# merbanan/rtl_433

Hardware: NVIDIA H100
Metric: IQ MS/s end-to-end demod+slice (higher is better)
Workload: dtype u8/int16/int32 fixed point

## Files before the change

### rtl_433_b200/csrc/r433b_api.cu

```cuda
#include <algorithm>
#include <cmath>
#include <cstdio>
#include <cstdlib>
#include <chrono>
#include <cstring>
#include <exception>
#include <atomic>
#include <mutex>
#include <string>
#include <thread>
#include <vector>

#include "../../include/r433b.h"
#include "../../include/r433b_abi.h"
#include "r433b_kernels.cuh"
#include "r433b_host.hpp"
#include "r433b_pulses.hpp"
#include "r433b_analyze.cuh"
#include "r433b_analyze_host.hpp"
#include "r433b_grab.cuh"

using namespace r433b;

#ifdef R433B_SIMT_EMU
#define R4_LAUNCH(kernel, grid, block, smem, stream, ...) simt::launch(dim3(grid), dim3(block), (size_t)(smem), kernel, __VA_ARGS__)
#else
#define R4_LAUNCH(kernel, grid, block, smem, stream, ...) kernel<<<(grid), (block), (smem), (stream)>>>(__VA_ARGS__)
#endif

static_assert(sizeof(struct bitbuffer) == 6604, "bitbuffer_t layout");
static_assert(sizeof(struct pulse_data) == 9672, "pulse_data_t layout");
static_assert(sizeof(struct r_device) == 152, "r_device layout");
static_assert(offsetof(struct bitbuffer, bb) == 204, "bitbuffer_t.bb offset");

namespace {

struct DevBuf {
    void *p = nullptr;
    size_t cap = 0;
};

struct HostBuf {
    void *p = nullptr;
    size_t cap = 0;
};

}

struct r433b_ctx {
    int device = 0;
    std::string err;
    std::mutex err_mu;
    int use_mag = 0;
    float level_limit = 0.0f, min_level = -12.1442f, min_snr = 9.0f, fm_low_pass = 0.0f;
    std::vector<r433b_device> devs;
    std::vector<r433b_gate> gates;
    r433b_batch batch{};
    std::vector<uint64_t> offsets, lengths;
    bool processed = false, fetched = false;
    unsigned fpdm = 0;
    int enable_fm = 0;
    int n_sms = 132;
    int spoil_front = 0;
    size_t min_caps[3] = {0, 0, 0};
    Levels lv{};
    DevBuf d_data, d_offsets, d_train, d_pkgs, d_ppool, d_gpool, d_counters, d_am, d_fm;
    DevBuf d_devparams, d_lists, d_pairs, d_arena, d_cursor;
    size_t pkg_cap = 0, pool_cap = 0, arena_cap = 0;
    unsigned n_ook = 0, n_fsk = 0;
    unsigned n_pkgs = 0, pool_used = 0;
    unsigned long long event_bytes = 0, n_events = 0, n_samples = 0, n_gated = 0;
    HostBuf h_pkgs, h_ppool, h_gpool, h_pairs, h_events;
    r433b_timing timing{};
    cudaEvent_t ev[6]{};
    int pipeline_groups = 0;
    cudaStream_t s_in = nullptr, s_det = nullptr, s_out = nullptr;
    static constexpr int kMaxGroups = 16;
    cudaEvent_t ev_in[kMaxGroups]{}, ev_det[kMaxGroups]{}, ev_slc[kMaxGroups]{}, ev_t[4 * kMaxGroups]{}, ev_f[kMaxGroups]{}, ev_init = nullptr;
    DevBuf d_order;
    DevBuf d_sort, d_copy;
    DevBuf d_ranges, d_state, d_lengths, d_stage, d_raw, d_log, d_amoff, d_chunks, d_tiles;
    std::vector<uint64_t> am_offsets;
    HostBuf h_ranges;
    bool d2h_done = false;
    bool pulse_mode = false;
    std::vector<PulseSet::Meta> pulse_meta;
    std::vector<uint32_t> dev_index;
    bool analyzed = false;
    std::vector<r433b_analysis> an;
    std::vector<r433b_guess> an_guess;
    std::vector<std::string> an_text;
    std::vector<r433b_pair> an_pairs;
    std::vector<uint8_t> an_events;
    DevBuf d_an, d_an_dev, d_an_gap, d_an_pairs, d_an_arena;
    std::thread worker;
    bool in_flight = false;
    int worker_rc = 0;
    r433b_batch sub_batch{};
    std::vector<uint64_t> sub_offsets, sub_lengths;
    r433b_results sub_res{};
    uint8_t const *grab_src = nullptr;
    unsigned grab_flip = 0;
    std::vector<uint32_t> p_events;
    std::vector<uint8_t> dispatched;
    std::vector<r433b_grab> grabs;
    std::vector<int64_t> grab_newest;
    bool grab_planned = false;
    uint64_t grab_pushed = 0;
    uint64_t grab_prior_bytes = 0;
    std::vector<uint64_t> grab_cum;
    DevBuf d_grab_prior, d_grab_segs, d_grab_stage;
    bool chained = false;
    std::vector<uint64_t> chain_base;
    std::vector<r433b_chain *> chains;
};

struct ChainSettings {
    uint32_t sample_format, samp_rate, center_frequency, fpdm, block_bytes;
    int use_mag, enable_fm;
    float level_limit, min_level, min_snr, fm_low_pass;
    bool operator==(ChainSettings const &o) const
    {
        return sample_format == o.sample_format && samp_rate == o.samp_rate && center_frequency == o.center_frequency
                && fpdm == o.fpdm && block_bytes == o.block_bytes && use_mag == o.use_mag && enable_fm == o.enable_fm
                && level_limit == o.level_limit && min_level == o.min_level && min_snr == o.min_snr
                && fm_low_pass == o.fm_low_pass;
    }
};

struct r433b_chain {
    r433b_ctx *ctx = nullptr;
    uint32_t n = 0;
    DevBuf d_state, d_train, d_state_copy, d_train_copy, d_flags, d_base;
    std::vector<uint8_t> open;
    std::vector<uint64_t> next;
    std::vector<uint64_t> base;
    ChainSettings settings{};
};

struct r433b_pulses {
    PulseSet set;
};

namespace {
void chain_free_device(r433b_chain *ch)
{
    for (DevBuf *b : {&ch->d_state, &ch->d_train, &ch->d_state_copy, &ch->d_train_copy, &ch->d_flags, &ch->d_base}) {
        if (b->p) cudaFree(b->p);
        b->p = nullptr;
        b->cap = 0;
    }
}
}

namespace {

int fail(r433b_ctx *c, int code, char const *what, cudaError_t e = cudaSuccess)
{
    if (c) {
        std::lock_guard<std::mutex> lock(c->err_mu);
        c->err = what;
        if (e != cudaSuccess) {
            c->err += ": ";
            c->err += cudaGetErrorString(e);
        }
    }
    return code;
}

#define CU(call)                                                   \
    do {                                                           \
        cudaError_t e_ = (call);                                   \
        if (e_ != cudaSuccess) return fail(ctx, R433B_ECUDA, #call, e_); \
    } while (0)

unsigned dp_flip_of(uint32_t sample_format) { return sample_format == R433B_FMT_CS8 ? 0x80808080u : 0u; }

int dev_reserve(r433b_ctx *ctx, DevBuf &b, size_t bytes)
{
    if (bytes <= b.cap) return 0;
    if (b.p) cudaFree(b.p);
    b.p = nullptr;
    b.cap = 0;
#ifdef R433B_EXACT_ALLOC
    size_t want = bytes;
#else
    size_t want = bytes + bytes / 8 + 256;
#endif
    cudaError_t e = cudaMalloc(&b.p, want);
    if (e != cudaSuccess) return fail(ctx, R433B_ENOMEM, "cudaMalloc", e);
    b.cap = want;
    return 0;
}

int host_reserve(r433b_ctx *ctx, HostBuf &b, size_t bytes)
{
    if (bytes <= b.cap) return 0;
    if (b.p) cudaFreeHost(b.p);
    b.p = nullptr;
    b.cap = 0;
    size_t want = bytes + bytes / 8 + 256;
    cudaError_t e = cudaMallocHost(&b.p, want);
    if (e != cudaSuccess) return fail(ctx, R433B_ENOMEM, "cudaMallocHost", e);
    b.cap = want;
    return 0;
}

}

extern "C" {

int r433b_create(int cuda_device, r433b_ctx **out)
{
    if (!out) return R433B_EINVAL;
    *out = nullptr;
    int n = 0;
    cudaError_t e = cudaGetDeviceCount(&n);
    if (e != cudaSuccess || n <= 0 || cuda_device < 0 || cuda_device >= n) {
        fprintf(stderr, "r433b_create: no usable CUDA device %d (%s); there is no CPU fallback\n", cuda_device,
                e != cudaSuccess ? cudaGetErrorString(e) : "device count is 0 or index out of range");
        return R433B_ECUDA;
    }
    r433b_ctx *ctx = new (std::nothrow) r433b_ctx();
    if (!ctx) return R433B_ENOMEM;
    ctx->device = cuda_device;
    if (cudaSetDevice(cuda_device) != cudaSuccess) {
        delete ctx;
        return R433B_ECUDA;
    }
    cudaFuncSetAttribute((void const *)k_front<2>, cudaFuncAttributePreferredSharedMemoryCarveout, 100);
    cudaFuncSetAttribute((void const *)k_front<4>, cudaFuncAttributePreferredSharedMemoryCarveout, 100);
    cudaFuncSetAttribute((void const *)k_detect<2>, cudaFuncAttributePreferredSharedMemoryCarveout, 100);
    cudaFuncSetAttribute((void const *)k_detect<4>, cudaFuncAttributePreferredSharedMemoryCarveout, 100);
    cudaFuncSetAttribute((void const *)k_slice2, cudaFuncAttributePreferredSharedMemoryCarveout,
                         (int)((kSliceCtasPerSm * (sizeof(g_slice_win) + sizeof(g_slice_seg) + 1024) * 100 + 228 * 1024 - 1) / (228 * 1024)));
    for (auto &v : ctx->ev) cudaEventCreate(&v);
    cudaStreamCreateWithFlags(&ctx->s_in, cudaStreamNonBlocking);
    cudaStreamCreateWithFlags(&ctx->s_det, cudaStreamNonBlocking);
    cudaStreamCreateWithFlags(&ctx->s_out, cudaStreamNonBlocking);
    for (auto &v : ctx->ev_in) cudaEventCreateWithFlags(&v, cudaEventDisableTiming);
    for (auto &v : ctx->ev_det) cudaEventCreateWithFlags(&v, cudaEventDisableTiming);
    for (auto &v : ctx->ev_slc) cudaEventCreateWithFlags(&v, cudaEventDisableTiming);
    for (auto &v : ctx->ev_t) cudaEventCreate(&v);
    for (auto &v : ctx->ev_f) cudaEventCreate(&v);
    cudaEventCreateWithFlags(&ctx->ev_init, cudaEventDisableTiming);
    ctx->lv = compute_levels(0, 0.0f, -12.1442f, 9.0f);
    if (char const *v = getenv("R433B_SPOIL_FRONT")) ctx->spoil_front = atoi(v);
    if (char const *v = getenv("R433B_TEST_CAPS")) {
        unsigned long long c[3] = {0, 0, 0};
        sscanf(v, "%llu,%llu,%llu", &c[0], &c[1], &c[2]);
        for (int i = 0; i < 3; ++i) ctx->min_caps[i] = (size_t)c[i];
    }
    if (cudaDeviceGetAttribute(&ctx->n_sms, cudaDevAttrMultiProcessorCount, cuda_device) != cudaSuccess || ctx->n_sms <= 0)
        ctx->n_sms = 132;
    *out = ctx;
    return R433B_OK;
}

void r433b_destroy(r433b_ctx *ctx)
{
    if (!ctx) return;
    if (ctx->worker.joinable()) ctx->worker.join();
    cudaSetDevice(ctx->device);
    for (r433b_chain *ch : ctx->chains) {
        chain_free_device(ch);
        ch->ctx = nullptr;
    }
    for (DevBuf *b : {&ctx->d_data, &ctx->d_offsets, &ctx->d_train, &ctx->d_pkgs, &ctx->d_ppool, &ctx->d_gpool,
                 &ctx->d_counters, &ctx->d_am, &ctx->d_fm, &ctx->d_devparams, &ctx->d_lists, &ctx->d_pairs,
                 &ctx->d_arena, &ctx->d_cursor, &ctx->d_ranges, &ctx->d_state, &ctx->d_lengths, &ctx->d_stage, &ctx->d_raw, &ctx->d_log, &ctx->d_amoff, &ctx->d_chunks, &ctx->d_tiles,
                 &ctx->d_order, &ctx->d_sort, &ctx->d_copy, &ctx->d_an, &ctx->d_an_dev, &ctx->d_an_gap, &ctx->d_an_pairs, &ctx->d_an_arena,
                 &ctx->d_grab_prior, &ctx->d_grab_segs, &ctx->d_grab_stage})
        if (b->p) cudaFree(b->p);
    for (HostBuf *b : {&ctx->h_pkgs, &ctx->h_ppool, &ctx->h_gpool, &ctx->h_pairs, &ctx->h_events, &ctx->h_ranges})
        if (b->p) cudaFreeHost(b->p);
    for (auto &v : ctx->ev)
        if (v) cudaEventDestroy(v);
    for (auto *arr : {ctx->ev_in, ctx->ev_det, ctx->ev_slc})
        for (int i = 0; i < r433b_ctx::kMaxGroups; ++i)
            if (arr[i]) cudaEventDestroy(arr[i]);
    for (auto &v : ctx->ev_t)
        if (v) cudaEventDestroy(v);
    for (auto &v : ctx->ev_f)
        if (v) cudaEventDestroy(v);
    if (ctx->ev_init) cudaEventDestroy(ctx->ev_init);
    for (cudaStream_t st : {ctx->s_in, ctx->s_det, ctx->s_out})
        if (st) cudaStreamDestroy(st);
    delete ctx;
}

char const *r433b_last_error(r433b_ctx const *ctx) { return ctx ? ctx->err.c_str() : "no context"; }

int r433b_set_levels(r433b_ctx *ctx, int use_mag_est, float level_limit_db, float min_level_db, float min_snr_db)
{
    if (!ctx) return R433B_EINVAL;
    ctx->use_mag = use_mag_est ? 1 : 0;
    ctx->level_limit = level_limit_db;
    ctx->min_level = min_level_db;
    ctx->min_snr = min_snr_db;
    ctx->lv = compute_levels(ctx->use_mag, level_limit_db, min_level_db, min_snr_db);
    return R433B_OK;
}

int r433b_set_fm_low_pass(r433b_ctx *ctx, float v)
{
    if (!ctx) return R433B_EINVAL;
    ctx->fm_low_pass = v;
    return R433B_OK;
}

int r433b_set_pipeline(r433b_ctx *ctx, int groups)
{
    if (!ctx || groups < 0 || groups > r433b_ctx::kMaxGroups) return R433B_EINVAL;
    ctx->pipeline_groups = groups;
    return R433B_OK;
}

int r433b_set_devices(r433b_ctx *ctx, r433b_device const *devs, uint32_t n)
{
    if (!ctx || (n && !devs)) return R433B_EINVAL;
    ctx->devs.assign(devs, devs + n);
    ctx->gates.clear();
    return R433B_OK;
}

int r433b_set_gates(r433b_ctx *ctx, r433b_gate const *gates, uint32_t n)
{
    if (!ctx || (n && !gates)) return R433B_EINVAL;
    if (n && n != ctx->devs.size()) return fail(ctx, R433B_EINVAL, "r433b_set_gates: one gate per registered device");
    for (uint32_t i = 0; i < n; ++i)
        if (gates[i].code_single > 0 || gates[i].code_single < -4 || gates[i].code_multi > 0 || gates[i].code_multi < -4)
            return fail(ctx, R433B_EINVAL, "r433b_set_gates: codes are decode_fn returns 0 .. -4");
    ctx->gates.assign(gates, gates + n);
    return R433B_OK;
}

uint64_t r433b_get_gated(r433b_ctx const *ctx) { return ctx && ctx->processed ? ctx->n_gated : 0; }

int r433b_set_r_devices(r433b_ctx *ctx, struct r_device *const *devs, uint32_t n)
{
    if (!ctx || (n && !devs)) return R433B_EINVAL;
    ctx->devs.resize(n);
    ctx->gates.clear();
    for (uint32_t i = 0; i < n; ++i) {
        struct r_device const *d = devs[i];
        r433b_device &o = ctx->devs[i];
        o.modulation = d->modulation;
        o.short_width = d->short_width;
        o.long_width = d->long_width;
        o.reset_limit = d->reset_limit;
        o.gap_limit = d->gap_limit;
        o.sync_width = d->sync_width;
        o.tolerance = d->tolerance;
        o.priority = d->priority;
    }
    return R433B_OK;
}

namespace {

int upload_slicer_tables(r433b_ctx *ctx, std::vector<uint32_t> const &rates, cudaStream_t st)
{
    size_t const n_devs = ctx->devs.size();
    std::vector<SlicerParams> sp(rates.size() * n_devs);
    for (size_t g = 0; g < rates.size(); ++g)
        for (size_t i = 0; i < n_devs; ++i) {
            sp[g * n_devs + i] = scale_device(ctx->devs[i], rates[g]);
            if (!ctx->gates.empty()) sp[g * n_devs + i].gate = ctx->gates[i].min_bits;
        }
    std::vector<unsigned> lists = slice_list(ctx->devs, 1), fsk = slice_list(ctx->devs, 2);
    ctx->n_ook = (unsigned)lists.size();
    ctx->n_fsk = (unsigned)fsk.size();
    lists.insert(lists.end(), fsk.begin(), fsk.end());
    if (int r = dev_reserve(ctx, ctx->d_devparams, std::max<size_t>(1, sp.size()) * sizeof(SlicerParams))) return r;
    if (int r = dev_reserve(ctx, ctx->d_lists, (lists.size() + 1) * sizeof(unsigned))) return r;
    size_t const stage_threads = (size_t)ctx->n_sms * kSliceCtasPerSm * kSliceThreads;
    if (int r = dev_reserve(ctx, ctx->d_stage, stage_threads * kStageWords * sizeof(uint32_t))) return r;
    if (!sp.empty()) CU(cudaMemcpyAsync(ctx->d_devparams.p, sp.data(), sp.size() * sizeof(SlicerParams), cudaMemcpyHostToDevice, st));
    if (!lists.empty()) CU(cudaMemcpyAsync(ctx->d_lists.p, lists.data(), lists.size() * sizeof(unsigned), cudaMemcpyHostToDevice, st));
    return R433B_OK;
}

int reserve_sort(r433b_ctx *ctx, size_t pkgs, size_t pool_entries, cudaStream_t st)
{
    size_t const cap0 = ctx->d_sort.cap;
    if (int r = dev_reserve(ctx, ctx->d_sort, (4 * kLenBins + pkgs / 32 + 3) * sizeof(unsigned))) return r;
    if (ctx->d_sort.cap != cap0) CU(cudaMemsetAsync(ctx->d_sort.p, 0, 2 * kLenBins * sizeof(unsigned), st));
    return dev_reserve(ctx, ctx->d_copy, (pool_entries + 2 * 32 * (size_t)kMaxPulses) * sizeof(PulseGap));
}

void launch_slice(r433b_ctx *ctx, GroupRange *range, unsigned n_pkgs, unsigned rate_index, cudaStream_t st)
{
    SortScratch ss;
    ss.hist = (unsigned *)ctx->d_sort.p;
    ss.fill = ss.hist + 2 * kLenBins;
    ss.base = ss.fill + 2 * kLenBins;
    ss.copy = (PulseGap *)ctx->d_copy.p;
    ss.copy_cap = std::min<size_t>(ctx->d_copy.cap / sizeof(PulseGap), 0xffffffffu);
    unsigned const n_devs = (unsigned)ctx->devs.size();
    r433b_package *pkgs = (r433b_package *)ctx->d_pkgs.p;
    SliceParams q{};
    q.pkgs = pkgs;
    q.range = range;
    q.order = (unsigned const *)ctx->d_order.p;
    q.copy = ss.copy;
    q.group_base = ss.base;
    q.dev = (SlicerParams const *)ctx->d_devparams.p + (size_t)rate_index * n_devs;
    q.n_devs = n_devs;
    q.ook_list = (unsigned const *)ctx->d_lists.p;
    q.fsk_list = q.ook_list + ctx->n_ook;
    q.n_ook = ctx->n_ook;
    q.n_fsk = ctx->n_fsk;
    q.pairs = (r433b_pair *)ctx->d_pairs.p;
    q.arena = (uint8_t *)ctx->d_arena.p;
    q.arena_cap = ctx->arena_cap;
    q.cursor = (unsigned long long *)ctx->d_cursor.p;
    q.stage = (uint32_t *)ctx->d_stage.p;
    unsigned const bgrid = (unsigned)ctx->n_sms * 2;
    R4_LAUNCH(k_bucket_count, bgrid, kBucketThreads, 0, st, range, pkgs, n_pkgs, n_devs, ss.hist);
    R4_LAUNCH(k_bucket_scan, 1, 32, 0, st, range, ss);
    R4_LAUNCH(k_bucket_scatter, bgrid, kBucketThreads, 0, st, range, (r433b_package const *)pkgs, n_pkgs, (unsigned *)ctx->d_order.p, ss,
              (int const *)ctx->d_ppool.p, (int const *)ctx->d_gpool.p);
    R4_LAUNCH(k_slice2, (unsigned)ctx->n_sms * kSliceCtasPerSm, kSliceThreads, 0, st, q);
}

int slice_ranges(r433b_ctx *ctx, std::vector<GroupRange> const &ranges, unsigned n_pkgs, size_t pool_entries, cudaStream_t st)
{
    unsigned const n_devs = (unsigned)ctx->devs.size();
    unsigned long long cursor[4] = {0, 0, 0, 0};
    ctx->timing.slice_launches = 0;
    CU(cudaEventRecord(ctx->ev[2], st));
    if (n_pkgs && n_devs) {
        size_t const pair_bytes = (size_t)n_pkgs * n_devs * sizeof(r433b_pair);
        if (int r = dev_reserve(ctx, ctx->d_pairs, pair_bytes)) return r;
        if (int r = dev_reserve(ctx, ctx->d_order, (size_t)n_pkgs * sizeof(unsigned))) return r;
        if (int r = reserve_sort(ctx, n_pkgs, pool_entries, st)) return r;
        if (int r = dev_reserve(ctx, ctx->d_ranges, ranges.size() * sizeof(GroupRange))) return r;
        if (int r = dev_reserve(ctx, ctx->d_cursor, 64)) return r;
        for (int attempt = 0; attempt < 3; ++attempt) {
            if (int r = dev_reserve(ctx, ctx->d_arena, ctx->arena_cap)) return r;
            CU(cudaMemsetAsync(ctx->d_pairs.p, 0, pair_bytes, st));
            CU(cudaMemsetAsync(ctx->d_cursor.p, 0, 64, st));
            CU(cudaMemcpyAsync(ctx->d_ranges.p, ranges.data(), ranges.size() * sizeof(GroupRange), cudaMemcpyHostToDevice, st));
            for (size_t g = 0; g < ranges.size(); ++g) {
                launch_slice(ctx, (GroupRange *)ctx->d_ranges.p + g, n_pkgs, (unsigned)g, st);
                CU(cudaGetLastError());
                ctx->timing.slice_launches++;
            }
            CU(cudaMemcpyAsync(cursor, ctx->d_cursor.p, sizeof(cursor), cudaMemcpyDeviceToHost, st));
            CU(cudaStreamSynchronize(st));
            if (!cursor[2]) break;
            ctx->arena_cap = (size_t)cursor[0] + (1u << 20);
            if (attempt == 2) return fail(ctx, R433B_EOVERFLOW, "event arena overflow");
        }
    }
    CU(cudaEventRecord(ctx->ev[3], st));
    CU(cudaEventSynchronize(ctx->ev[3]));
    cudaEventElapsedTime(&ctx->timing.slice_ms, ctx->ev[2], ctx->ev[3]);
    ctx->event_bytes = cursor[0];
    ctx->n_events = cursor[1];
    ctx->n_gated = cursor[3];
    return R433B_OK;
}

int process_iq(r433b_ctx *ctx, r433b_batch const *b, r433b_chain *ch, uint8_t const *last)
{
    if (!ctx || !b || !b->offsets || (b->n_streams && !b->data)) return fail(ctx, R433B_EINVAL, "null argument");
    if (b->sample_format != R433B_FMT_CU8 && b->sample_format != R433B_FMT_CS16 && b->sample_format != R433B_FMT_CS8
            && b->sample_format != R433B_FMT_CF32)
        return fail(ctx, R433B_EINVAL, "sample_format must be R433B_FMT_CU8, _CS8, _CS16 or _CF32");
    bool const cf32 = b->sample_format == R433B_FMT_CF32;
    unsigned const in_div = cf32 ? 2 : 1;
    if (b->samp_rate == 0) return fail(ctx, R433B_EINVAL, "samp_rate is 0");
    int const SS = (int)(b->sample_format & 0xff);
    uint32_t block_bytes = b->block_bytes ? b->block_bytes : 262144u;
    int const T = kTile;
    if (block_bytes % (uint32_t)(T * SS) != 0) return fail(ctx, R433B_EINVAL, "block_bytes must be a multiple of 2048 samples (4096 bytes of cu8, 8192 of cs16)");
    for (uint32_t i = 0; i <= b->n_streams; ++i) {
        if (b->offsets[i] % (16 * in_div)) return fail(ctx, R433B_EINVAL, "stream offsets must be multiples of 16 bytes (32 for cf32)");
        if (i && b->offsets[i] < b->offsets[i - 1]) return fail(ctx, R433B_EINVAL, "offsets not ascending");
    }
    int enable_fm = 0;
    for (auto const &d : ctx->devs)
        if (d.modulation >= 16) enable_fm = 1;
    unsigned const fpdm = b->fpdm_mode == R433B_FPDM_AUTO ? (b->center_frequency > 800000000u ? 1u : 0u) : b->fpdm_mode;
    ChainSettings const settings{b->sample_format, b->samp_rate, b->center_frequency, fpdm, block_bytes, ctx->use_mag, enable_fm,
                                 ctx->level_limit, ctx->min_level, ctx->min_snr, ctx->fm_low_pass};
    if (ch) {
        if (ch->ctx != ctx || !last) return fail(ctx, R433B_EINVAL, "r433b_process_chained: chain of another context, or no last[]");
        if (b->n_streams != ch->n) return fail(ctx, R433B_EINVAL, "r433b_process_chained: n_streams differs from the chain's");
        if (std::find(ch->open.begin(), ch->open.end(), 1) != ch->open.end() && !(settings == ch->settings))
            return fail(ctx, R433B_ESTATE, "r433b_process_chained: format, rate, frequency, block size, levels or FM "
                                           "settings changed while a file of the chain is open");
        for (uint32_t i = 0; i < b->n_streams; ++i) {
            uint64_t const in_bytes = b->lengths ? b->lengths[i] : b->offsets[i + 1] - b->offsets[i];
            if (!last[i] && in_bytes % ((uint64_t)block_bytes * in_div))
                return fail(ctx, R433B_EINVAL, "r433b_process_chained: a chunk that is not its file's last must be whole "
                                               "blocks (block_bytes, 2 x block_bytes of cf32 input)");
        }
    }
    CU(cudaSetDevice(ctx->device));
    ctx->processed = ctx->fetched = false;
    ctx->chained = false;
    ctx->pulse_mode = false;
    ctx->batch = *b;
    ctx->batch.sample_format = (uint32_t)SS;
    ctx->batch.block_bytes = block_bytes;
    ctx->offsets.assign(b->offsets, b->offsets + b->n_streams + 1);
    for (auto &v : ctx->offsets) v /= in_div;
    ctx->batch.offsets = ctx->offsets.data();
    ctx->lengths.resize(b->n_streams);
    for (uint32_t i = 0; i < b->n_streams; ++i) {
        uint64_t gap = b->offsets[i + 1] - b->offsets[i];
        ctx->lengths[i] = b->lengths ? b->lengths[i] : gap;
        if (ctx->lengths[i] > gap) return fail(ctx, R433B_EINVAL, "lengths[i] exceeds the gap to the next offset");
        if (cf32) ctx->lengths[i] = ctx->lengths[i] / 8 * 4;
    }
    ctx->batch.lengths = ctx->lengths.data();
    ctx->grabs.clear();
    ctx->grab_planned = false;
    ctx->timing.grab_ms = 0;
    uint64_t const total_bytes = b->n_streams ? b->offsets[b->n_streams] / in_div : 0;
    uint64_t used_bytes = 0;
    for (uint64_t v : ctx->lengths) used_bytes += v;
    uint32_t const n_devs = (uint32_t)ctx->devs.size();

    ctx->fpdm = fpdm;
    ctx->enable_fm = enable_fm;

    cudaStream_t const st = 0;
    ctx->d2h_done = false;

    uint8_t const *d_in;
    if (b->data_on_device && !cf32) {
        d_in = (uint8_t const *)b->data;
    } else {
        if (int r = dev_reserve(ctx, ctx->d_data, total_bytes + 64)) return r;
        d_in = (uint8_t const *)ctx->d_data.p;
    }
    ctx->grab_src = d_in;
    ctx->grab_flip = dp_flip_of(b->sample_format);
    if (cf32 && !b->data_on_device)
        if (int r = dev_reserve(ctx, ctx->d_raw, 2 * total_bytes + 64)) return r;
    if (int r = dev_reserve(ctx, ctx->d_offsets, (b->n_streams + 1) * sizeof(uint64_t))) return r;
    CU(cudaMemcpy(ctx->d_offsets.p, ctx->offsets.data(), (b->n_streams + 1) * sizeof(uint64_t), cudaMemcpyHostToDevice));
    if (int r = dev_reserve(ctx, ctx->d_lengths, std::max<size_t>(1, b->n_streams) * sizeof(uint64_t))) return r;
    if (b->n_streams) CU(cudaMemcpy(ctx->d_lengths.p, ctx->lengths.data(), b->n_streams * sizeof(uint64_t), cudaMemcpyHostToDevice));
    if (int r = dev_reserve(ctx, ctx->d_train, (size_t)std::max(1u, b->n_streams) * kTrainInts * sizeof(int))) return r;
    if (int r = dev_reserve(ctx, ctx->d_log, (size_t)std::max(1u, b->n_streams) * kLogCap * 2 * sizeof(unsigned))) return r;
    if (int r = dev_reserve(ctx, ctx->d_counters, 64)) return r;
    if (int r = dev_reserve(ctx, ctx->d_cursor, 64)) return r;
    ctx->am_offsets.resize(b->n_streams + 1);
    ctx->am_offsets[0] = 0;
    for (uint32_t i = 0; i < b->n_streams; ++i)
        ctx->am_offsets[i + 1] = ctx->am_offsets[i] + (ctx->lengths[i] / SS + T - 1) / T * T;
    uint64_t const am_samples = ctx->am_offsets[b->n_streams];
    if (int r = dev_reserve(ctx, ctx->d_am, am_samples * sizeof(int16_t) + 16)) return r;
    if (int r = dev_reserve(ctx, ctx->d_chunks, am_samples / kChunk * sizeof(ChunkInfo) + 16)) return r;
    if (int r = dev_reserve(ctx, ctx->d_tiles, am_samples / T * sizeof(TileInfo) + 16)) return r;
    if (int r = dev_reserve(ctx, ctx->d_amoff, (b->n_streams + 1) * sizeof(uint64_t))) return r;
    CU(cudaMemcpy(ctx->d_amoff.p, ctx->am_offsets.data(), (b->n_streams + 1) * sizeof(uint64_t), cudaMemcpyHostToDevice));
    if (b->want_stages)
        if (int r = dev_reserve(ctx, ctx->d_fm, total_bytes / SS * sizeof(int16_t) + 16)) return r;

    DetectParams dp{};
// ... 1287 lines not shown
```

### rtl_433_b200/csrc/r433b_host.hpp

```cpp
#pragma once
#include <algorithm>
#include <cmath>
#include <cstdint>
#include <cstring>
#include <vector>

#include "../../include/r433b.h"
#include "../../include/r433b_abi.h"
#include "r433b_core.cuh"
#include "r433b_slice.cuh"

namespace r433b {

inline Levels compute_levels(int use_mag, float level_limit, float min_level, float min_snr)
{
    Levels lv;
    if (use_mag) {
        lv.fixed_high = level_limit < 0.0 ? (int)(powf(10, (level_limit + 84.2884f) / 20.0f)) : 0;
        lv.min_high = (int)(powf(10, (min_level + 84.2884f) / 20.0f));
        lv.ratio = (int)(0.5 + powf(10, min_snr / 20.0f));
    } else {
        lv.fixed_high = level_limit < 0.0 ? (int)(powf(10, (level_limit + 42.1442f) / 10.0f)) : 0;
        lv.min_high = (int)(powf(10, (min_level + 42.1442f) / 10.0f));
        lv.ratio = (int)(0.5 + powf(10, min_snr / 10.0f));
    }
    lv.max_high = (int)(powf(10, (0 + 42.1442f) / 10.0f));
    return lv;
}

inline void fm_coeffs(int cs16, uint32_t rate, float low_pass, int &a1, int &b0)
{
    if (low_pass > 1e4f)
        low_pass = low_pass / rate;
    else if (low_pass >= 1.0f)
        low_pass = 1e6f / low_pass / rate;
    double ita = 1.0 / tan(M_PI_2 * low_pass);
    if (!cs16) {
        double gain = 1.0 / (1.0 + ita) / 2;
        a1 = (int)((ita - 1.0) * gain * 32768);
        b0 = (int)(gain * 32768);
    } else {
        double gain = 1.0 / (1.0 + ita);
        a1 = (int)((ita - 1.0) * gain * (1 << 30));
        b0 = (int)(gain * (1 << 30));
    }
}

inline SlicerParams scale_device(r433b_device const &d, uint32_t rate)
{
    SlicerParams t{};
    float per_us = rate / 1.0e6f;
    t.modulation = (int)d.modulation;
    t.s_short = d.short_width * per_us;
    t.s_long = d.long_width * per_us;
    t.s_reset = d.reset_limit * per_us;
    t.s_gap = d.gap_limit * per_us;
    t.s_sync = d.sync_width * per_us;
    t.s_tol = d.tolerance * per_us;
    bool bad3 = (d.short_width > 0 && t.s_short <= 0) || (d.long_width > 0 && t.s_long <= 0)
            || (d.reset_limit > 0 && t.s_reset <= 0);
    bool bad6 = bad3 || (d.gap_limit > 0 && t.s_gap <= 0) || (d.sync_width > 0 && t.s_sync <= 0)
            || (d.tolerance > 0 && t.s_tol <= 0);
    t.ok = (bad6 ? 0 : 1) | (bad3 ? 0 : 2);
    if ((int)d.modulation == kModOokRzi) {
        t.s_gap = t.s_sync = t.s_tol = 0;
    }
    t.f_short = d.short_width > 0.0f ? 1.0f / (d.short_width * per_us) : 0;
    t.f_long = d.long_width > 0.0f ? 1.0f / (d.long_width * per_us) : 0;
    t.priority = d.priority;
    return t;
}


inline std::vector<unsigned> slice_list(std::vector<r433b_device> const &devs, int package_type)
{
    std::vector<unsigned> v;
    for (unsigned i = 0; i < (unsigned)devs.size(); ++i)
        if (device_takes((int)devs[i].modulation, package_type)) v.push_back(i);
    std::sort(v.begin(), v.end(), [&](unsigned a, unsigned c) {
        r433b_device const &x = devs[a], &y = devs[c];
        if (x.modulation != y.modulation) return x.modulation < y.modulation;
        if (x.reset_limit != y.reset_limit) return x.reset_limit < y.reset_limit;
        if (x.short_width != y.short_width) return x.short_width < y.short_width;
        return a < c;
    });
    return v;
}


struct EventHead {
    uint32_t num_rows, dirty, free_row, len;
};

inline EventHead event_head(uint32_t h)
{
    if ((h & 0xff) == 0xff) return {1, 0, 1, 1};
    return {h & 0x7f, (h >> 7) & 1, (h >> 8) & 0xff, h >> 16};
}

template <class Row>
inline int event_rows(uint32_t const *ev, EventHead const &e, Row &&row)
{
    uint32_t const end = e.len;
    uint32_t const h = ev[0];
    if ((h & 0xff) == 0xff) {
        uint32_t const data = h >> 16, bits = (h >> 8) & 31;
        if (bits > 16) return -1;
        row(0u, bits, (h >> 13) & 7, &data, bits ? 1u : 0u);
        return 1;
    }
    uint32_t q = 1;
    for (uint32_t r = 0; r < e.num_rows && r < R433B_BITBUF_ROWS; ++r) {
        if (q + 1 > end) return -1;
        uint32_t const w = ev[q];
        q += 1;
        if (w >> 31) {
            uint32_t const data = w & 0xffff, bits = (w >> 16) & 31;
            if (bits > 16) return -1;
            row(r, bits, (w >> 21) & 0x3ff, &data, bits ? 1u : 0u);
            continue;
        }
        uint32_t const bits = w & 0xffff;
        uint32_t words = (bits + 31) / 32;
        if (e.dirty && r + 1 == e.num_rows) words = ev[end - 1];
        if (q + words > end) return -1;
        row(r, bits, w >> 16, ev + q, words);
        q += words;
    }
    return (int)q;
}

inline int event_to_bitbuffer(uint8_t const *ev8, uint32_t pair_bytes, uint32_t index, struct bitbuffer *out,
        uint32_t *consumed)
{
    if (!ev8 || !out || (pair_bytes & 3)) return -1;
    uint32_t const *ev = reinterpret_cast<uint32_t const *>(ev8);
    uint32_t const total = pair_bytes / 4;
    uint32_t pos = 0;
    EventHead e;
    for (uint32_t i = 0;; ++i) {
        if (pos + 1 > total) return -1;
        e = event_head(ev[pos]);
        if (e.len < 1 || pos + e.len > total) return -1;
        if (i == index) break;
        pos += e.len;
    }
    memset(out, 0, sizeof(*out));
    out->num_rows = (uint16_t)e.num_rows;
    out->free_row = (uint16_t)e.free_row;
    uint8_t *flat = &out->bb[0][0];
    int const rc = event_rows(ev + pos, e, [&](uint32_t r, uint32_t bits, uint32_t syncs, uint32_t const *data, uint32_t words) {
        out->bits_per_row[r] = (uint16_t)bits;
        out->syncs_before_row[r] = (uint16_t)syncs;
        size_t at = (size_t)r * R433B_BITBUF_COLS;
        size_t room = sizeof(out->bb) - at;
        size_t nb = (size_t)words * 4;
        memcpy(flat + at, data, nb < room ? nb : room);
    });
    if (rc < 0) return -1;
    if (consumed) *consumed = (pos + e.len) * 4;
    return 0;
}

inline int event_long_form(uint32_t const *ev, EventHead const &e, std::vector<uint32_t> &out)
{
    size_t const at = out.size();
    out.push_back(0);
    int const q = event_rows(ev, e, [&](uint32_t, uint32_t bits, uint32_t syncs, uint32_t const *data, uint32_t words) {
        out.push_back(bits | (syncs << 16));
        out.insert(out.end(), data, data + words);
    });
    if (q < 0) return -1;
    out.insert(out.end(), ev + q, ev + e.len);
    out[at] = e.num_rows | (e.dirty << 7) | (e.free_row << 8) | ((uint32_t)(out.size() - at) << 16);
    return 0;
}

}
```

### rtl_433_b200/csrc/r433b_kernels.cuh

```cuda
#pragma once
#include <cuda_runtime.h>
#include <stdint.h>

#include "../../include/r433b.h"
#include "r433b_core.cuh"
#include "r433b_slice.cuh"
#include "r433b_detect.cuh"

namespace r433b {


__global__ void k_cf32_to_cs16(float4 const *in, uint2 *out, size_t n4)
{
    for (size_t i = (size_t)blockIdx.x * blockDim.x + threadIdx.x; i < n4; i += (size_t)gridDim.x * blockDim.x) {
        float4 v = __ldcs(in + i);
        float f[4] = {v.x, v.y, v.z, v.w};
        int s[4];
#pragma unroll
        for (int k = 0; k < 4; ++k) {
            float t = __fmul_rn(f[k], 32767.0f);
            int q = (t >= -2147483648.0f && t < 2147483648.0f) ? __float2int_rz(t) : (int)0x80000000;
            q = q < -32767 ? -32767 : (q > 32767 ? 32767 : q);
            s[k] = q;
        }
// ... 9 lines not shown
    unsigned pkg_begin, pkg_end;
    unsigned pool_begin, pool_end;
    unsigned long long arena_begin, arena_end;
    unsigned long long events_end, gated_end;
    unsigned overflow;
    unsigned next;
    unsigned count[2], groups[2];
};

__global__ void k_mark(GroupRange *r, int which, unsigned const *counters, unsigned long long const *cursor)
{
    if (which == 0) {
        r->pkg_begin = counters[0];
        r->pool_begin = counters[1];
    } else if (which == 1) {
        r->pkg_end = counters[0];
        r->pool_end = counters[1];
        r->overflow = counters[2];
        r->next = 0;
    } else if (which == 2) {
        r->arena_begin = cursor[0];
    } else {
        r->arena_end = cursor[0];
        r->events_end = cursor[1];
        r->gated_end = cursor[3];
        r->overflow |= (unsigned)cursor[2] << 1;
    }
}

constexpr unsigned kLenBins = kMaxPulses + 1;

__host__ __device__ inline unsigned len_bin(unsigned num_pulses) { return num_pulses < kLenBins ? num_pulses : kMaxPulses; }
__host__ __device__ inline unsigned copy_rows(unsigned len) { return len < (unsigned)kMaxPulses ? len + 1 : kMaxPulses; }

struct SortScratch {
    unsigned *hist;
    unsigned *fill;
    unsigned *base;
    PulseGap *copy;
    unsigned long long copy_cap;
};

constexpr int kBucketThreads = 256;
__global__ void __launch_bounds__(kBucketThreads) k_bucket_count(GroupRange *r, r433b_package *pkgs, unsigned n_pkgs, unsigned n_devs, unsigned *hist)
{
    unsigned const b0 = r->pkg_begin, b1 = r->pkg_end < n_pkgs ? r->pkg_end : n_pkgs;
    for (unsigned pk = b0 + blockIdx.x * kBucketThreads + threadIdx.x; pk < b1; pk += gridDim.x * kBucketThreads) {
        r433b_package const k = pkgs[pk];
        pkgs[pk].first_pair = pk * n_devs;
        atomicAdd(&hist[(k.type == 1 ? 0 : kLenBins) + len_bin(k.num_pulses)], 1u);
    }
}

__global__ void __launch_bounds__(32) k_bucket_scan(GroupRange *r, SortScratch s)
{
    constexpr unsigned kBins = 2 * kLenBins, kPer = (kBins + 31) / 32;
    __shared__ unsigned hist[kPer * 32];
    unsigned const lane = threadIdx.x;
    auto len = [](unsigned i) { return i < kLenBins ? kMaxPulses - i : kLenBins + kMaxPulses - i; };
    for (unsigned i = lane; i < kPer * 32; i += 32) hist[i] = i < kBins ? s.hist[(i < kLenBins ? 0 : kLenBins) + len(i)] : 0;
    __syncwarp();
    unsigned n0 = 0, n1 = 0;
    for (unsigned j = 0; j < kPer; ++j) {
        unsigned const i = lane * kPer + j;
        (i < kLenBins ? n0 : n1) += hist[i];
    }
    unsigned at = n0 + n1;
#pragma unroll
    for (int o = 1; o < 32; o <<= 1) {
        unsigned const v = __shfl_up_sync(0xffffffffu, at, o);
        if ((int)lane >= o) at += v;
    }
    at -= n0 + n1;
#pragma unroll
    for (int o = 16; o > 0; o >>= 1) {
        n0 += __shfl_xor_sync(0xffffffffu, n0, o);
        n1 += __shfl_xor_sync(0xffffffffu, n1, o);
    }
    unsigned const g0 = (n0 + 31) / 32, g1 = (n1 + 31) / 32;
    unsigned long long e = 0;
    for (unsigned j = 0, a = at; j < kPer; ++j) {
        unsigned const i = lane * kPer + j, n = hist[i];
        unsigned const q = a - (i < kLenBins ? 0 : n0);
        e += (unsigned long long)((q + n + 31) / 32 - (q + 31) / 32) * 32 * copy_rows(len(i));
        a += n;
    }
    unsigned long long incl = e;
#pragma unroll
    for (int o = 1; o < 32; o <<= 1) {
        unsigned long long const v = __shfl_up_sync(0xffffffffu, incl, o);
        if ((int)lane >= o) incl += v;
    }
    unsigned long long const total = __shfl_sync(0xffffffffu, incl, 31);
    bool const fits = total <= s.copy_cap;
    e = incl - e;
    for (unsigned j = 0; j < kPer; ++j) {
        unsigned const i = lane * kPer + j, n = hist[i];
        if (i >= kBins) break;
        unsigned const t = i < kLenBins ? 0 : 1, b = t * kLenBins + len(i), q = at - (t ? n0 : 0);
        s.fill[b] = at;
        if (n) s.hist[b] = 0;
        unsigned const size = 32 * copy_rows(len(i));
        for (unsigned g = (q + 31) / 32; g * 32 < q + n; ++g, e += size) s.base[(t ? g0 : 0) + g] = (unsigned)e;
        at += n;
    }
    if (lane == 0) {
        s.base[g0 + g1] = (unsigned)total;
        r->count[0] = n0;
        r->count[1] = n1;
        r->groups[0] = fits ? g0 : 0;
        r->groups[1] = fits ? g1 : 0;
        if (!fits) r->overflow |= 4;
        r->next = 0;
    }
}

__global__ void __launch_bounds__(kBucketThreads) k_bucket_scatter(GroupRange *r, r433b_package const *pkgs, unsigned n_pkgs, unsigned *order,
                                                                  SortScratch s, int const *pulse_pool, int const *gap_pool)
{
    unsigned const lane = threadIdx.x & 31;
    unsigned const b0 = r->pkg_begin, b1 = r->pkg_end < n_pkgs ? r->pkg_end : n_pkgs;
    unsigned const n0 = r->count[0], g0 = r->groups[0], g1 = r->groups[1];
    for (unsigned w = b0 + blockIdx.x * kBucketThreads + threadIdx.x - lane; w < b1; w += gridDim.x * kBucketThreads) {
        unsigned const pk = w + lane;
        unsigned dst = 0, rows = 0, off = 0;
        if (pk < b1) {
            r433b_package const k = pkgs[pk];
            unsigned const t = k.type == 1 ? 0 : 1, len = len_bin(k.num_pulses);
            unsigned const pos = atomicAdd(&s.fill[t * kLenBins + len], 1u);
            order[b0 + pos] = pk;
            unsigned const q = pos - (t ? n0 : 0);
            if (q / 32 < (t ? g1 : g0)) {
                dst = s.base[(t ? g0 : 0) + q / 32] + q % 32;
                rows = copy_rows(len);
                off = k.pulse_off;
            }
        }
        for (int l = 0; l < 32; ++l) {
            unsigned const n = __shfl_sync(0xffffffffu, rows, l), d = __shfl_sync(0xffffffffu, dst, l);
            unsigned const o = __shfl_sync(0xffffffffu, off, l);
            for (unsigned k = lane; k < n; k += 32) s.copy[d + 32 * k] = PulseGap{pulse_pool[o + k], gap_pool[o + k]};
        }
    }
}

struct SliceParams {
    r433b_package const *pkgs;
    GroupRange *range;
    unsigned const *order;
    PulseGap const *copy;
    unsigned const *group_base;
    SlicerParams const *dev;
    unsigned n_devs;
    unsigned const *ook_list, *fsk_list;
    unsigned n_ook, n_fsk;
    r433b_pair *pairs;
    uint8_t *arena;
    unsigned long long arena_cap;
    unsigned long long *cursor;
    uint32_t *stage;
};

constexpr int kSliceThreads = 128;
constexpr unsigned kStageWords = 1024;
constexpr int kSliceCtasPerSm = 8;

__shared__ uint32_t g_slice_win[kSliceWindow][kSliceThreads];
__shared__ unsigned g_slice_seg[2][kSliceThreads];
struct SliceWindow {
    static constexpr bool kOn = true;
    __device__ __forceinline__ static uint32_t &slot(unsigned s) { return g_slice_win[s][threadIdx.x]; }
};

__global__ void __launch_bounds__(kSliceThreads, kSliceCtasPerSm) k_slice2(SliceParams p)
{
    unsigned const lane = threadIdx.x & 31, warp = threadIdx.x >> 5;
    GroupRange const *rg = p.range;
    unsigned const pk_begin = rg->pkg_begin;
    unsigned const groups_ook = rg->groups[0], groups_fsk = rg->groups[1];
    unsigned const items_ook = p.n_ook * groups_ook, items = items_ook + p.n_fsk * groups_fsk;
    uint32_t *stage = p.stage + ((size_t)blockIdx.x * kSliceThreads + threadIdx.x) * kStageWords;
    for (;;) {
        unsigned item = 0;
        if (lane == 0) item = atomicAdd(&p.range->next, 1u);
        item = __shfl_sync(0xffffffffu, item, 0);
        if (item >= items) break;
        int const t = item < items_ook ? 0 : 1;
        unsigned const rel = t ? item - items_ook : item;
        unsigned const groups = t ? groups_fsk : groups_ook;
        unsigned const slot = rel / groups;
        unsigned const g = rel - slot * groups;
        unsigned const dev = (t ? p.fsk_list : p.ook_list)[slot];
        unsigned const in_type = g * 32 + lane;
        bool const active = in_type < rg->count[t];
        unsigned const pk = active ? p.order[pk_begin + (t ? rg->count[0] : 0) + in_type] : 0;
        SlicerParams const sp = p.dev[dev];
        PulseViewT<32> pv;
        pv.w = p.copy + p.group_base[(t ? groups_ook : 0) + g] + lane;
        pv.n = active ? len_bin(p.pkgs[pk].num_pulses) : 0;
        unsigned bytes = 0, nev = 0, ng1 = 0, ngN = 0, wb = 0;
        if (active) {
            EventWriterT<SliceWindow> w;
            w.init(stage, kStageWords, (unsigned)sp.gate);
            slice_dispatch(pv, sp, w);
            bytes = w.committed * 4;
            wb = w.wb;
            nev = w.events;
            ng1 = w.gated1;
            ngN = w.gatedN;
        }
        unsigned incl = bytes;
#pragma unroll
        for (int o = 1; o < 32; o <<= 1) {
            unsigned v = __shfl_up_sync(0xffffffffu, incl, o);
            if ((int)lane >= o) incl += v;
        }
        unsigned const total = __shfl_sync(0xffffffffu, incl, 31);
        unsigned evs = nev, dropped = ng1 + ngN;
#pragma unroll
        for (int o = 16; o > 0; o >>= 1) {
            evs += __shfl_xor_sync(0xffffffffu, evs, o);
            dropped += __shfl_xor_sync(0xffffffffu, dropped, o);
        }
        unsigned long long wbase = 0;
        if (lane == 0 && total) {
            wbase = atomicAdd(p.cursor, (unsigned long long)total);
            atomicAdd(p.cursor + 1, (unsigned long long)evs);
        }
        if (lane == 0 && dropped) atomicAdd(p.cursor + 3, (unsigned long long)dropped);
        wbase = __shfl_sync(0xffffffffu, wbase, 0);
        unsigned long long const off = wbase + incl - bytes;
        bool const fits = off + bytes <= p.arena_cap;
        if (active && bytes && !fits) atomicOr(p.cursor + 2, 1ull);
        if (__all_sync(0xffffffffu, bytes <= kStageWords * 4)) {
            unsigned const first = (incl - bytes) / 4;
            g_slice_seg[0][threadIdx.x] = first;
            g_slice_seg[1][threadIdx.x] = first + wb;
            __syncwarp();
            unsigned const w0 = threadIdx.x - lane;
            unsigned n = total / 4;
            if (wbase + total > p.arena_cap) n = wbase >= p.arena_cap ? 0 : (unsigned)((p.arena_cap - wbase) / 4);
            unsigned const lead = (unsigned)(wbase / 4) & 31;
            uint32_t *to = reinterpret_cast<uint32_t *>(p.arena + wbase) - lead;
            uint32_t const *scratch = stage - (size_t)lane * kStageWords;
            for (unsigned j = lane; j < n + lead; j += 32) {
                if (j < lead) continue;
                unsigned const i = j - lead;
                unsigned l = 0;
#pragma unroll
                for (unsigned s = 16; s; s >>= 1)
                    if (g_slice_seg[0][w0 + l + s] <= i) l += s;
                unsigned const at = i - g_slice_seg[0][w0 + l];
                uint32_t const v = i >= g_slice_seg[1][w0 + l] ? g_slice_win[at % kSliceWindow][w0 + l]
                                                               : scratch[(size_t)l * kStageWords + at];
                __stcs(to + j, v);
            }
            __syncwarp();
        } else if (active && bytes && fits) {
            EventWriter w;
            w.init(reinterpret_cast<uint32_t *>(p.arena + off), bytes / 4, (unsigned)sp.gate);
            slice_dispatch(pv, sp, w);
        }
        if (active) {
            r433b_pair pr;
            pr.offset = off;
            pr.bytes = bytes;
            pr.events = nev;
            pr.gated_single = ng1;
            pr.gated_multi = ngN;
            p.pairs[(size_t)pk * p.n_devs + dev] = pr;
        }
    }
}

}
```

Before: 143,100.

## Deduplicate slicer devices with identical effective params and replicate outputs

On the host, devices whose slicer parameters normalize to the same key are grouped into equivalence classes per sample rate. The slice kernel runs once per class representative and copies the resulting event bytes and pair records to every member device, instead of running the slicer separately for each device. Slicer params are also staged in shared memory per warp. This removes redundant slicing work but adds replicated arena writes and depends on the key normalization matching slicer semantics exactly.

```diff
diff --git a/rtl_433_b200/csrc/r433b_api.cu b/rtl_433_b200/csrc/r433b_api.cu
--- a/rtl_433_b200/csrc/r433b_api.cu
+++ b/rtl_433_b200/csrc/r433b_api.cu
@@ -67,7 +67,11 @@
     DevBuf d_data, d_offsets, d_train, d_pkgs, d_ppool, d_gpool, d_counters, d_am, d_fm;
     DevBuf d_devparams, d_lists, d_pairs, d_arena, d_cursor;
     size_t pkg_cap = 0, pool_cap = 0, arena_cap = 0;
-    unsigned n_ook = 0, n_fsk = 0;
+    struct SliceLists {
+        size_t reps, begin, members;
+        unsigned n_ook, n_fsk;
+    };
+    std::vector<SliceLists> slice_lists;
     unsigned n_pkgs = 0, pool_used = 0;
     unsigned long long event_bytes = 0, n_events = 0, n_samples = 0, n_gated = 0;
     HostBuf h_pkgs, h_ppool, h_gpool, h_pairs, h_events;
@@ -233,7 +237,7 @@
     cudaFuncSetAttribute((void const *)k_detect<2>, cudaFuncAttributePreferredSharedMemoryCarveout, 100);
     cudaFuncSetAttribute((void const *)k_detect<4>, cudaFuncAttributePreferredSharedMemoryCarveout, 100);
     cudaFuncSetAttribute((void const *)k_slice2, cudaFuncAttributePreferredSharedMemoryCarveout,
-                         (int)((kSliceCtasPerSm * (sizeof(g_slice_win) + sizeof(g_slice_seg) + 1024) * 100 + 228 * 1024 - 1) / (228 * 1024)));
+                         (int)((kSliceCtasPerSm * (sizeof(g_slice_win) + sizeof(g_slice_seg) + sizeof(g_slice_sp) + 1024) * 100 + 228 * 1024 - 1) / (228 * 1024)));
     for (auto &v : ctx->ev) cudaEventCreate(&v);
     cudaStreamCreateWithFlags(&ctx->s_in, cudaStreamNonBlocking);
     cudaStreamCreateWithFlags(&ctx->s_det, cudaStreamNonBlocking);
@@ -368,10 +372,22 @@
             sp[g * n_devs + i] = scale_device(ctx->devs[i], rates[g]);
             if (!ctx->gates.empty()) sp[g * n_devs + i].gate = ctx->gates[i].min_bits;
         }
-    std::vector<unsigned> lists = slice_list(ctx->devs, 1), fsk = slice_list(ctx->devs, 2);
-    ctx->n_ook = (unsigned)lists.size();
-    ctx->n_fsk = (unsigned)fsk.size();
-    lists.insert(lists.end(), fsk.begin(), fsk.end());
+    std::vector<unsigned> const ook = slice_list(ctx->devs, 1), fsk = slice_list(ctx->devs, 2);
+    std::vector<unsigned> lists;
+    ctx->slice_lists.clear();
+    for (size_t g = 0; g < rates.size(); ++g) {
+        SliceClasses c;
+        r433b_ctx::SliceLists l;
+        l.n_ook = add_slice_classes(c, ook, sp.data() + g * n_devs);
+        l.n_fsk = add_slice_classes(c, fsk, sp.data() + g * n_devs);
+        l.reps = lists.size();
+        lists.insert(lists.end(), c.reps.begin(), c.reps.end());
+        l.begin = lists.size();
+        lists.insert(lists.end(), c.begin.begin(), c.begin.end());
+        l.members = lists.size();
+        lists.insert(lists.end(), c.members.begin(), c.members.end());
+        ctx->slice_lists.push_back(l);
+    }
     if (int r = dev_reserve(ctx, ctx->d_devparams, std::max<size_t>(1, sp.size()) * sizeof(SlicerParams))) return r;
     if (int r = dev_reserve(ctx, ctx->d_lists, (lists.size() + 1) * sizeof(unsigned))) return r;
     size_t const stage_threads = (size_t)ctx->n_sms * kSliceCtasPerSm * kSliceThreads;
@@ -407,10 +423,12 @@
     q.group_base = ss.base;
     q.dev = (SlicerParams const *)ctx->d_devparams.p + (size_t)rate_index * n_devs;
     q.n_devs = n_devs;
-    q.ook_list = (unsigned const *)ctx->d_lists.p;
-    q.fsk_list = q.ook_list + ctx->n_ook;
-    q.n_ook = ctx->n_ook;
-    q.n_fsk = ctx->n_fsk;
+    r433b_ctx::SliceLists const &l = ctx->slice_lists[rate_index];
+    q.reps = (unsigned const *)ctx->d_lists.p + l.reps;
+    q.member_begin = (unsigned const *)ctx->d_lists.p + l.begin;
+    q.members = (unsigned const *)ctx->d_lists.p + l.members;
+    q.n_ook = l.n_ook;
+    q.n_fsk = l.n_fsk;
     q.pairs = (r433b_pair *)ctx->d_pairs.p;
     q.arena = (uint8_t *)ctx->d_arena.p;
     q.arena_cap = ctx->arena_cap;
diff --git a/rtl_433_b200/csrc/r433b_host.hpp b/rtl_433_b200/csrc/r433b_host.hpp
--- a/rtl_433_b200/csrc/r433b_host.hpp
+++ b/rtl_433_b200/csrc/r433b_host.hpp
@@ -1,8 +1,10 @@
 #pragma once
 #include <algorithm>
+#include <array>
 #include <cmath>
 #include <cstdint>
 #include <cstring>
+#include <map>
 #include <vector>
 
 #include "../../include/r433b.h"
@@ -71,6 +73,61 @@
     return t;
 }
 
+inline SlicerParams slicer_key(SlicerParams t)
+{
+    t.priority = 0;
+    int const m = t.modulation;
+    int const fam = m == kModFskPwm ? (int)kModOokPwm : m == kModFskPcm ? (int)kModOokPcm : m == kModFskMc ? (int)kModOokMc : m;
+    bool const runs = fam == kModOokRzi ? (t.ok & 2) && t.s_long != 0
+                                        : (t.ok & 1) && !(fam == kModOokPcm && t.s_long == 0) && !(fam == kModOokNrzs && t.s_short == 0);
+    if (!runs) {
+        SlicerParams z{};
+        z.modulation = m;
+        return z;
+    }
+    t.ok = 1;
+    switch (fam) {
+    case kModOokPcm:
+        t.s_sync = 0;
+        if (!t.s_gap) t.s_gap = t.s_reset;
+        if (t.s_tol <= 0) t.s_tol = t.s_long / 4;
+        break;
+    case kModOokPpm:
+        t.f_short = t.f_long = 0;
+        if (t.s_tol > 0) t.s_gap = 0;
+        else t.s_sync = t.s_tol = 0;
+        break;
+    case kModOokPwm:
+        t.f_short = t.f_long = 0;
+        if (t.s_tol <= 0) t.s_tol = 0;
+        break;
+    case kModOokMc:
+        t.s_long = t.s_gap = t.s_sync = 0;
+        t.f_short = t.f_long = 0;
+        if (t.s_tol <= 0) t.s_tol = 0;
+        break;
+    case kModOokDmc: case kModOokPiwmDc:
+        t.s_gap = t.s_sync = 0;
+        t.f_short = t.f_long = 0;
+        break;
+    case kModOokPiwmRaw:
+        t.s_gap = t.s_sync = 0;
+        t.f_long = 0;
+        break;
+    case kModOokNrzs: case kModOokOsv1:
+        t.s_long = t.s_gap = t.s_sync = t.s_tol = 0;
+        t.f_short = t.f_long = 0;
+        break;
+    case kModOokRzi:
+        t.s_gap = t.s_sync = t.s_tol = 0;
+        t.f_short = t.f_long = 0;
+        break;
+    default:
+        break;
+    }
+    return t;
+}
+
 
 inline std::vector<unsigned> slice_list(std::vector<r433b_device> const &devs, int package_type)
 {
@@ -85,6 +142,32 @@
         return a < c;
     });
     return v;
+}
+
+struct SliceClasses {
+    std::vector<unsigned> reps, begin{0}, members;
+};
+
+inline unsigned add_slice_classes(SliceClasses &c, std::vector<unsigned> const &list, SlicerParams const *sp)
+{
+    static_assert(sizeof(SlicerParams) == 12 * sizeof(uint32_t), "SlicerParams: twelve words, no padding");
+    using Key = std::array<uint32_t, 12>;
+    std::map<Key, unsigned> index;
+    std::vector<std::vector<unsigned>> cls;
+    for (unsigned d : list) {
+        SlicerParams const k = slicer_key(sp[d]);
+        Key key;
+        std::memcpy(key.data(), &k, sizeof k);
+        auto const it = index.emplace(key, (unsigned)cls.size()).first;
+        if (it->second == cls.size()) cls.emplace_back();
+        cls[it->second].push_back(d);
+    }
+    for (auto const &m : cls) {
+        c.reps.push_back(m[0]);
+        c.members.insert(c.members.end(), m.begin(), m.end());
+        c.begin.push_back((unsigned)c.members.size());
+    }
+    return (unsigned)cls.size();
 }
 
 
diff --git a/rtl_433_b200/csrc/r433b_kernels.cuh b/rtl_433_b200/csrc/r433b_kernels.cuh
--- a/rtl_433_b200/csrc/r433b_kernels.cuh
+++ b/rtl_433_b200/csrc/r433b_kernels.cuh
@@ -185,7 +185,7 @@
     unsigned const *group_base;
     SlicerParams const *dev;
     unsigned n_devs;
-    unsigned const *ook_list, *fsk_list;
+    unsigned const *reps, *member_begin, *members;
     unsigned n_ook, n_fsk;
     r433b_pair *pairs;
     uint8_t *arena;
@@ -200,6 +200,7 @@
 
 __shared__ uint32_t g_slice_win[kSliceWindow][kSliceThreads];
 __shared__ unsigned g_slice_seg[2][kSliceThreads];
+__shared__ SlicerParams g_slice_sp[kSliceThreads / 32];
 struct SliceWindow {
     static constexpr bool kOn = true;
     __device__ __forceinline__ static uint32_t &slot(unsigned s) { return g_slice_win[s][threadIdx.x]; }
@@ -223,11 +224,15 @@
         unsigned const groups = t ? groups_fsk : groups_ook;
         unsigned const slot = rel / groups;
         unsigned const g = rel - slot * groups;
-        unsigned const dev = (t ? p.fsk_list : p.ook_list)[slot];
+        unsigned const cls = (t ? p.n_ook : 0) + slot;
+        unsigned const dev = p.reps[cls];
         unsigned const in_type = g * 32 + lane;
         bool const active = in_type < rg->count[t];
         unsigned const pk = active ? p.order[pk_begin + (t ? rg->count[0] : 0) + in_type] : 0;
-        SlicerParams const sp = p.dev[dev];
+        __syncwarp();
+        if (lane == 0) g_slice_sp[warp] = p.dev[dev];
+        __syncwarp();
+        SlicerParams const &sp = g_slice_sp[warp];
         PulseViewT<32> pv;
         pv.w = p.copy + p.group_base[(t ? groups_ook : 0) + g] + lane;
         pv.n = active ? len_bin(p.pkgs[pk].num_pulses) : 0;
@@ -255,15 +260,16 @@
             evs += __shfl_xor_sync(0xffffffffu, evs, o);
             dropped += __shfl_xor_sync(0xffffffffu, dropped, o);
         }
+        unsigned const m_begin = p.member_begin[cls], m = p.member_begin[cls + 1] - m_begin;
         unsigned long long wbase = 0;
         if (lane == 0 && total) {
-            wbase = atomicAdd(p.cursor, (unsigned long long)total);
-            atomicAdd(p.cursor + 1, (unsigned long long)evs);
-        }
-        if (lane == 0 && dropped) atomicAdd(p.cursor + 3, (unsigned long long)dropped);
+            wbase = atomicAdd(p.cursor, (unsigned long long)m * total);
+            atomicAdd(p.cursor + 1, (unsigned long long)m * evs);
+        }
+        if (lane == 0 && dropped) atomicAdd(p.cursor + 3, (unsigned long long)m * dropped);
         wbase = __shfl_sync(0xffffffffu, wbase, 0);
         unsigned long long const off = wbase + incl - bytes;
-        bool const fits = off + bytes <= p.arena_cap;
+        bool const fits = off + (unsigned long long)(m - 1) * total + bytes <= p.arena_cap;
         if (active && bytes && !fits) atomicOr(p.cursor + 2, 1ull);
         if (__all_sync(0xffffffffu, bytes <= kStageWords * 4)) {
             unsigned const first = (incl - bytes) / 4;
@@ -271,39 +277,49 @@
             g_slice_seg[1][threadIdx.x] = first + wb;
             __syncwarp();
             unsigned const w0 = threadIdx.x - lane;
-            unsigned n = total / 4;
-            if (wbase + total > p.arena_cap) n = wbase >= p.arena_cap ? 0 : (unsigned)((p.arena_cap - wbase) / 4);
-            unsigned const lead = (unsigned)(wbase / 4) & 31;
-            uint32_t *to = reinterpret_cast<uint32_t *>(p.arena + wbase) - lead;
             uint32_t const *scratch = stage - (size_t)lane * kStageWords;
-            for (unsigned j = lane; j < n + lead; j += 32) {
-                if (j < lead) continue;
-                unsigned const i = j - lead;
-                unsigned l = 0;
-#pragma unroll
-                for (unsigned s = 16; s; s >>= 1)
-                    if (g_slice_seg[0][w0 + l + s] <= i) l += s;
-                unsigned const at = i - g_slice_seg[0][w0 + l];
-                uint32_t const v = i >= g_slice_seg[1][w0 + l] ? g_slice_win[at % kSliceWindow][w0 + l]
-                                                               : scratch[(size_t)l * kStageWords + at];
-                __stcs(to + j, v);
+            for (unsigned mj = 0; mj < m; ++mj) {
+                unsigned long long const mbase = wbase + (unsigned long long)mj * total;
+                unsigned n = total / 4;
+                if (mbase + total > p.arena_cap) n = mbase >= p.arena_cap ? 0 : (unsigned)((p.arena_cap - mbase) / 4);
+                unsigned const lead = (unsigned)(mbase / 4) & 31;
+                uint32_t *to = reinterpret_cast<uint32_t *>(p.arena + mbase) - lead;
+                for (unsigned j = lane; j < n + lead; j += 32) {
+                    if (j < lead) continue;
+                    unsigned const i = j - lead;
+                    unsigned l = 0;
+#pragma unroll
+                    for (unsigned s = 16; s; s >>= 1)
+                        if (g_slice_seg[0][w0 + l + s] <= i) l += s;
+                    unsigned const at = i - g_slice_seg[0][w0 + l];
+                    uint32_t const v = i >= g_slice_seg[1][w0 + l] ? g_slice_win[at % kSliceWindow][w0 + l]
+                                                                   : scratch[(size_t)l * kStageWords + at];
+                    __stcs(to + j, v);
+                }
             }
             __syncwarp();
         } else if (active && bytes && fits) {
+            uint32_t *out = reinterpret_cast<uint32_t *>(p.arena + off);
             EventWriter w;
-            w.init(reinterpret_cast<uint32_t *>(p.arena + off), bytes / 4, (unsigned)sp.gate);
+            w.init(out, bytes / 4, (unsigned)sp.gate);
             slice_dispatch(pv, sp, w);
+            for (unsigned mj = 1; mj < m; ++mj) {
+                uint32_t *to = reinterpret_cast<uint32_t *>(p.arena + off + (unsigned long long)mj * total);
+                for (unsigned i = 0; i < bytes / 4; ++i) to[i] = out[i];
+            }
         }
         if (active) {
             r433b_pair pr;
-            pr.offset = off;
             pr.bytes = bytes;
             pr.events = nev;
             pr.gated_single = ng1;
             pr.gated_multi = ngN;
-            p.pairs[(size_t)pk * p.n_devs + dev] = pr;
-        }
-    }
-}
-
-}
+            for (unsigned mj = 0; mj < m; ++mj) {
+                pr.offset = off + (unsigned long long)mj * total;
+                p.pairs[(size_t)pk * p.n_devs + p.members[m_begin + mj]] = pr;
+            }
+        }
+    }
+}
+
+}
```

After: 144,300 (median of 6 runs). About the same (+0.8%).
